# jipolanco/PencilArrays.jl

Hardware: NVIDIA H100
Metric: transpose_GiB_per_s (higher is better)
Workload: dtype c128 (bytes; pure data movement)

## Files before the change

pencilarrays.jl_b200/csrc/fft.cu:

```cuda
#include <cuda_runtime.h>

#include <algorithm>
#include <cmath>
#include <map>
#include <mutex>
#include <tuple>
#include <type_traits>
#include <vector>

#ifndef PA_FFT_TWIDDLE_LOOKUPS
#define PA_FFT_TWIDDLE_LOOKUPS 1
#endif
#include "fft_core.hpp"
#include "flags.cuh"
#include "pa_internal.hpp"

namespace pa {

using pa_fft::cplx;
using pa_fft::cplx_t;

template <class T>
struct Vec2;
template <>
struct Vec2<double> {
  using type = double2;
};
template <>
struct Vec2<float> {
  using type = float2;
};
__device__ __forceinline__ double2 vec2(double x, double y) { return make_double2(x, y); }
__device__ __forceinline__ float2 vec2(float x, float y) { return make_float2(x, y); }

template <class T, int STRIDE = 1>
struct Twiddles {
  const typename Vec2<T>::type* tab;
  __device__ __forceinline__ cplx_t<T> operator()(int k) const {
    const typename Vec2<T>::type w = __ldg(tab + STRIDE * k);
    return cplx_t<T>{w.x, w.y};
  }
};

constexpr int FFT_MAXB = 8;
constexpr int FFT_MAXO = PA_MAX_DIMS - 2;
constexpr int FFT_THREADS = 256;
constexpr int fft_lines(int logL) { return logL >= 10 ? 4 : 8; }
constexpr int fft_lines_f32(int logL) { return logL >= 10 ? 8 : 16; }

struct FftBlock {
  const char* src;
  int y0, ey;
  long long ssy;
  long long ssx;
  long long so[FFT_MAXO];
};
struct FftParams {
  int nb;
  FftBlock blk[FFT_MAXB];
  char* dst;
  long long ex;
  long long dsx;
  int no;
  long long oe[FFT_MAXO], dso[FFT_MAXO];
  int L, logL, sign, pitch;
  int linear;
  const void* tw;
  unsigned tiles_x;
  const void* tw4;
  int sine;
};

template <class T>
struct SmLine {
  cplx_t<T>* p;
  __device__ __forceinline__ cplx_t<T> get(int i) const { return p[pa_fft::pad_index(i)]; }
  __device__ __forceinline__ void put(int i, cplx_t<T> v) { p[pa_fft::pad_index(i)] = v; }
};

template <int LOGM>
struct PassRadix {
  static constexpr int LOGR = (LOGM % 3 == 0) ? 3 : (LOGM % 3);
};

template <int LOGL, int LOGM, int C, class T, class Tw>
__device__ __forceinline__ void fft_passes(cplx_t<T>* sm, int pitch, int ncol, int sign, const Tw& tw) {
  if constexpr (LOGM > 0) {
    constexpr int LOGR = PassRadix<LOGM>::LOGR;
    constexpr int R = 1 << LOGR, L = 1 << LOGL, M = 1 << LOGM;
    constexpr int PER_LINE = L / R;
    constexpr int TOTAL = C * PER_LINE;
#pragma unroll
    for (int w0 = 0; w0 < TOTAL; w0 += FFT_THREADS) {
      const int w = w0 + (int)threadIdx.x;
      const int c = w / PER_LINE, u = w % PER_LINE;
      if (w < TOTAL && c < ncol) {
        SmLine<T> x{sm + c * pitch};
        pa_fft::butterfly<R>(x, u, L, M, sign, tw);
      }
    }
    __syncthreads();
    fft_passes<LOGL, LOGM - LOGR, C>(sm, pitch, ncol, sign, tw);
  }
}

template <int LOGL, int LOGM>
__device__ __forceinline__ int fft_pos(int k) {
  if constexpr (LOGM == 0) {
    return 0;
  } else {
    constexpr int LOGR = PassRadix<LOGM>::LOGR;
    return ((k & ((1 << LOGR) - 1)) << (LOGM - LOGR)) + fft_pos<LOGL, LOGM - LOGR>(k >> LOGR);
  }
}

template <int LOGL, class T>
__device__ __forceinline__ T out_real(const T* line, int i) {
  return line[2 * pa_fft::pad_index(fft_pos<LOGL, LOGL>(i >> 1)) + (i & 1)];
}

template <int C, class T>
__device__ __forceinline__ void gather_rows(const FftParams& p, const long long* so_off, long long x0,
                                            int c, int r, int ncol, cplx_t<T>* line) {
  using V = typename Vec2<T>::type;
  constexpr int RS = FFT_THREADS / C;
  constexpr int U = 8;
#pragma unroll
  for (int b = 0; b < FFT_MAXB; ++b) {
    if (b < p.nb) {
      const FftBlock& B = p.blk[b];
      const char* s = B.src + so_off[b] + (x0 + c) * B.ssx;
      const int ey = B.ey, y0 = B.y0;
      const long long ssy = B.ssy;
      for (int y = r; y < ey; y += U * RS) {
        V v[U];
#pragma unroll
        for (int k = 0; k < U; ++k) {
          const int yy = y + k * RS;
          if (c < ncol && yy < ey) v[k] = __ldcs(reinterpret_cast<const V*>(s + (long long)yy * ssy));
        }
#pragma unroll
        for (int k = 0; k < U; ++k) {
          const int yy = y + k * RS;
          if (c < ncol && yy < ey) line[pa_fft::pad_index(y0 + yy)] = cplx_t<T>{v[k].x, v[k].y};
        }
      }
    }
  }
}

enum class RealMap {
  rfft,
  dct2,
  dct3,
};

template <RealMap MAP, int LOGL, class T>
__device__ __forceinline__ void put_real(T* line, int n, T x, bool sine) {
  constexpr int L = 1 << LOGL, N = 2 * L;
  if constexpr (MAP == RealMap::rfft) {
    line[2 * pa_fft::pad_index(n >> 1) + (n & 1)] = x;
  } else if constexpr (MAP == RealMap::dct2) {
    const int i = (n & 1) ? N - 1 - (n >> 1) : (n >> 1);
    line[2 * pa_fft::pad_index(i >> 1) + (i & 1)] = ((n & 1) && sine) ? -x : x;
  } else {
    const int j = sine ? N - 1 - n : n;
    if (j <= L) line[2 * pa_fft::pad_index(j)] = x;
    if (j >= L) line[2 * pa_fft::pad_index(N - j) + 1] = x;
  }
}

template <int C, class T, class Put>
__device__ __forceinline__ void gather_real_rows(const FftParams& p, const long long* so_off, long long x0,
                                                 int c, int r, int ncol, const Put& put) {
  constexpr int RS = FFT_THREADS / C;
  constexpr int U = 8;
#pragma unroll
  for (int b = 0; b < FFT_MAXB; ++b) {
    if (b < p.nb) {
      const FftBlock& B = p.blk[b];
      const char* s = B.src + so_off[b] + (x0 + c) * B.ssx;
      const int ey = B.ey, y0 = B.y0;
      const long long ssy = B.ssy;
      for (int y = r; y < ey; y += U * RS) {
        T v[U];
#pragma unroll
        for (int k = 0; k < U; ++k) {
          const int yy = y + k * RS;
          if (c < ncol && yy < ey) v[k] = __ldcs(reinterpret_cast<const T*>(s + (long long)yy * ssy));
        }
#pragma unroll
        for (int k = 0; k < U; ++k) {
          const int yy = y + k * RS;
          if (c < ncol && yy < ey) put(y0 + yy, v[k]);
        }
      }
    }
  }
}

__device__ __forceinline__ long long cta_offsets(const FftParams& p, int C, long long* so_off,
                                                 long long* d_off) {
  unsigned long long bid = blockIdx.x;
  const long long x0 = (long long)(bid % p.tiles_x) * C;
  bid /= p.tiles_x;
#pragma unroll
  for (int b = 0; b < FFT_MAXB; ++b) so_off[b] = 0;
  *d_off = 0;
#pragma unroll 1
  for (int i = 0; i < p.no; ++i) {
    const long long k = (long long)(bid % (unsigned long long)p.oe[i]);
    bid /= (unsigned long long)p.oe[i];
    *d_off += k * p.dso[i];
#pragma unroll
    for (int b = 0; b < FFT_MAXB; ++b)
      if (b < p.nb) so_off[b] += k * p.blk[b].so[i];
  }
  return x0;
}

template <int LOGL, int C, class T>
struct FftCtaShape {
  static constexpr int RS = FFT_THREADS / C;
  static constexpr int LOGRS = (C == 16) ? 4 : (C == 8) ? 5 : 6;
  static_assert((1 << LOGRS) == RS, "rows per sweep");
  static constexpr int LOGR1 = (sizeof(T) == 8 && C == 4 && LOGL > LOGRS) ? (LOGL - LOGRS) : 0;
  static_assert(LOGR1 == 0 || LOGL - LOGR1 == LOGRS, "first-pass stride must equal the sweep");
  static_assert(LOGR1 <= 4, "the register first pass is at most radix 16");
};

template <int LOGL, int C, class T>
__device__ __forceinline__ void fft_cta_lines(const FftParams& p, const long long* so_off, long long x0,
                                              int ncol, cplx_t<T>* sm) {
  using cx = cplx_t<T>;
  using V = typename Vec2<T>::type;
  constexpr int L = 1 << LOGL;
  const int t = threadIdx.x;
  const int pitch = p.pitch;

  constexpr int RS = FftCtaShape<LOGL, C, T>::RS;
  constexpr int LOGR1 = FftCtaShape<LOGL, C, T>::LOGR1;
  const V* twp = reinterpret_cast<const V*>(p.tw);
  const Twiddles<T> tw{twp};
  {
    const int c = p.linear ? t / RS : t % C, r = p.linear ? t % RS : t / C;
    cx* line = sm + c * pitch;
    if constexpr (LOGR1 > 0) {
      constexpr int R1 = 1 << LOGR1;
      if (c < ncol) {
        V v[R1];
#pragma unroll
        for (int q = 0; q < R1; ++q) {
          const int y = r + q * RS;
          const char* s = nullptr;
#pragma unroll
          for (int b = 0; b < FFT_MAXB; ++b)
            if (b < p.nb && y >= p.blk[b].y0 && y < p.blk[b].y0 + p.blk[b].ey)
              s = p.blk[b].src + so_off[b] + (long long)(y - p.blk[b].y0) * p.blk[b].ssy +
                  (x0 + c) * p.blk[b].ssx;
          v[q] = __ldcs(reinterpret_cast<const V*>(s));
        }
        cx a[R1];
#pragma unroll
        for (int q = 0; q < R1; ++q) a[q] = cx{v[q].x, v[q].y};
        pa_fft::butterfly_regs<R1>(a, r, L, L, p.sign, tw);
#pragma unroll
        for (int q = 0; q < R1; ++q) line[pa_fft::pad_index(r + q * RS)] = a[q];
      }
    } else {
      gather_rows<C, T>(p, so_off, x0, c, r, ncol, line);
    }
  }
  __syncthreads();

  fft_passes<LOGL, LOGL - LOGR1, C>(sm, pitch, ncol, p.sign, tw);
}

template <int LOGL, int LOGR1>
__device__ __forceinline__ int fft_out_pos(int k) {
  return ((k & ((1 << LOGR1) - 1)) << (LOGL - LOGR1)) + fft_pos<LOGL, LOGL - LOGR1>(k >> LOGR1);
}

template <int LOGL, int C, class T>
__device__ __forceinline__ void unpack_fft_cta(const FftParams& p) {
  using cx = cplx_t<T>;
  using V = typename Vec2<T>::type;
  constexpr int L = 1 << LOGL;
  extern __shared__ __align__(16) unsigned char fft_smem[];
  cx* sm = reinterpret_cast<cx*>(fft_smem);
  const int t = threadIdx.x;
  long long so_off[FFT_MAXB], d_off;
  const long long x0 = cta_offsets(p, C, so_off, &d_off);
  const int ncol = (int)((p.ex - x0) < C ? (p.ex - x0) : C);
  const int pitch = p.pitch;
  constexpr int LOGR1 = FftCtaShape<LOGL, C, T>::LOGR1;

  fft_cta_lines<LOGL, C, T>(p, so_off, x0, ncol, sm);

  char* d = p.dst + x0 * p.dsx + d_off;
  for (int c = 0; c < ncol; ++c) {
    const cx* line = sm + c * pitch;
    V* out = reinterpret_cast<V*>(d + c * p.dsx);
#pragma unroll
    for (int k0 = 0; k0 < L; k0 += FFT_THREADS) {
      const int k = k0 + t;
      if (k < L) {
        const int pos = ((k & ((1 << LOGR1) - 1)) << (LOGL - LOGR1)) +
                        fft_pos<LOGL, LOGL - LOGR1>(k >> LOGR1);
        const cx v = line[pa_fft::pad_index(pos)];
        __stcs(out + k, vec2(v.x, v.y));
      }
    }
  }
}

template <int LOGL, int C, class T>
__global__ void __launch_bounds__(FFT_THREADS) k_unpack_fft(const __grid_constant__ FftParams p) {
  unpack_fft_cta<LOGL, C, T>(p);
}

struct FftGetParams {
  FftParams p;
  MultiFlags mf;
};
static_assert(sizeof(FftGetParams) <= 4096, "FftParams + MultiFlags must fit the kernel parameters");

template <int LOGL, int C, class T>
__global__ void __maxnreg__(128) k_get_fft(const __grid_constant__ FftGetParams gp) {
  const MultiFlags& mf = gp.mf;
  if (mf.ready.n > 0) {
    if ((int)threadIdx.x < mf.ready.n) {
      if (blockIdx.x < 8) flag_signal(mf.ready.remote[threadIdx.x], mf.ready.seq[threadIdx.x]);
      flag_wait(mf.ready.local[threadIdx.x], mf.ready.seq[threadIdx.x], mf.timeout_ns, mf.err);
    }
    __syncthreads();
  }
  unpack_fft_cta<LOGL, C, T>(gp.p);
  if (mf.done.n > 0) {
    __syncthreads();
    int last = 0;
    if (threadIdx.x == 0) {
      __threadfence_system();
      last = atomicAdd(mf.counter, 1u) == gridDim.x - 1;
      if (last) {
        *mf.counter = 0;
        __threadfence_system();
      }
    }
    if (__syncthreads_or(last) && (int)threadIdx.x < mf.done.n)
      flag_signal(mf.done.remote[threadIdx.x], mf.done.seq[threadIdx.x]);
  }
}

struct RfftParams {
  const char* src;
  char* dst;
  long long nlines;
  long long src_line, dst_line;
  int pitch;
  const void* tw;
};

template <int LOGL, int C, class T, class Out>
__device__ __forceinline__ void rfft_forward_tail(cplx_t<T>* sm, int pitch, int ncol, int t,
                                                  const typename Vec2<T>::type* twp, const Out& out) {
  using cx = cplx_t<T>;
  using V = typename Vec2<T>::type;
  constexpr int L = 1 << LOGL;
  constexpr int P = L / 2 + 1;
  const Twiddles<T> twN{twp};
  const Twiddles<T, 2> twL{twp};
  fft_passes<LOGL, LOGL, C>(sm, pitch, ncol, -1, twL);

#pragma unroll
  for (int w0 = 0; w0 < C * P; w0 += FFT_THREADS) {
    const int w = w0 + t, c = w / P, k = w % P;
    if (w < C * P && c < ncol) {
      const cx* line = sm + c * pitch;
      cx xk, xl;
      pa_fft::rfft_post_pair(line[pa_fft::pad_index(fft_pos<LOGL, LOGL>(k & (L - 1)))],
                             line[pa_fft::pad_index(fft_pos<LOGL, LOGL>((L - k) & (L - 1)))], twN(k),
                             &xk, &xl);
      V* o = reinterpret_cast<V*>(out(c));
      __stcs(o + k, vec2(xk.x, xk.y));
      if (k != L - k) __stcs(o + (L - k), vec2(xl.x, xl.y));
    }
  }
}

template <int LOGL, int C, bool UNROLL, class T>
__device__ __forceinline__ void brfft_pre(cplx_t<T>* sm, int pitch, int ncol, int t, const Twiddles<T>& twN) {
  using cx = cplx_t<T>;
  constexpr int L = 1 << LOGL;
  constexpr int P = L / 2 + 1;
  constexpr int TRIPS = (C * P + FFT_THREADS - 1) / FFT_THREADS;
#pragma unroll(UNROLL ? TRIPS : 1)
  for (int w0 = 0; w0 < C * P; w0 += FFT_THREADS) {
    const int w = w0 + t, c = w / P, k = w % P;
    if (w < C * P && c < ncol) {
      cx* line = sm + c * pitch;
      cx zk, zl;
      pa_fft::brfft_pre_pair(k, line[pa_fft::pad_index(k)], line[pa_fft::pad_index(L - k)], twN(k),
                             &zk, &zl);
      line[pa_fft::pad_index(k)] = zk;
      if (k > 0) line[pa_fft::pad_index(L - k)] = zl;
    }
  }
  __syncthreads();
}

template <int LOGL, int C, bool FWD, class T, class Src>
__device__ __forceinline__ void rfft_load(cplx_t<T>* sm, int pitch, int ncol, int t, const Src& src) {
  using cx = cplx_t<T>;
  using V = typename Vec2<T>::type;
  constexpr int L = 1 << LOGL;
  constexpr int RS = FFT_THREADS / C;
  constexpr int NIN = FWD ? L : L + 1;
  constexpr int U = (NIN + RS - 1) / RS;
  const int c = t / RS, r = t % RS;
  if (c < ncol) {
    const V* s = src(c);
    cx* line = sm + c * pitch;
    V v[U];
#pragma unroll
    for (int q = 0; q < U; ++q)
      if (r + q * RS < NIN) v[q] = __ldcs(s + r + q * RS);
#pragma unroll
    for (int q = 0; q < U; ++q)
      if (r + q * RS < NIN) line[pa_fft::pad_index(r + q * RS)] = cx{v[q].x, v[q].y};
  }
}

template <int LOGL, int C, bool FWD, class T>
__global__ void __launch_bounds__(FFT_THREADS) k_rfft(const __grid_constant__ RfftParams p) {
  using cx = cplx_t<T>;
  using V = typename Vec2<T>::type;
  constexpr int L = 1 << LOGL;
  extern __shared__ __align__(16) unsigned char fft_smem[];
  cx* sm = reinterpret_cast<cx*>(fft_smem);
  const int t = threadIdx.x;
  const long long l0 = (long long)blockIdx.x * C;
  const int ncol = (int)((p.nlines - l0) < C ? (p.nlines - l0) : C);
  const int pitch = p.pitch;
  const V* twp = reinterpret_cast<const V*>(p.tw);

  rfft_load<LOGL, C, FWD, T>(sm, pitch, ncol, t, [&p, l0](int c) {
    return reinterpret_cast<const V*>(p.src + (l0 + c) * p.src_line);
  });
  __syncthreads();

  if constexpr (FWD) {
    rfft_forward_tail<LOGL, C, T>(sm, pitch, ncol, t, twp,
                                  [&p, l0](int c) { return p.dst + (l0 + c) * p.dst_line; });
  } else {
    brfft_pre<LOGL, C, true, T>(sm, pitch, ncol, t, Twiddles<T>{twp});
    fft_passes<LOGL, LOGL, C>(sm, pitch, ncol, 1, Twiddles<T, 2>{twp});

#pragma unroll
    for (int w0 = 0; w0 < C * L; w0 += FFT_THREADS) {
      const int w = w0 + t, c = w >> LOGL, n = w & (L - 1);
      if (c < ncol) {
        const cx v = sm[c * pitch + pa_fft::pad_index(fft_pos<LOGL, LOGL>(n))];
        __stcs(reinterpret_cast<V*>(p.dst + (l0 + c) * p.dst_line) + n, vec2(v.x, v.y));
      }
    }
  }
}

template <int LOGL, int C, class T>
__global__ void __launch_bounds__(FFT_THREADS) k_unpack_brfft(const __grid_constant__ FftParams p) {
  using cx = cplx_t<T>;
  using V = typename Vec2<T>::type;
  constexpr int L = 1 << LOGL;
  constexpr int RS = FFT_THREADS / C;
  extern __shared__ __align__(16) unsigned char fft_smem[];
  cx* sm = reinterpret_cast<cx*>(fft_smem);
  const int t = threadIdx.x;
  long long so_off[FFT_MAXB], d_off;
  const long long x0 = cta_offsets(p, C, so_off, &d_off);
  const int ncol = (int)((p.ex - x0) < C ? (p.ex - x0) : C);
  const int pitch = p.pitch;
// ... 147 lines not shown
  cx* sm = reinterpret_cast<cx*>(fft_smem);
  const int t = threadIdx.x;
  const long long l0 = (long long)blockIdx.x * C;
  const int ncol = (int)((p.nlines - l0) < C ? (p.nlines - l0) : C);
  const int pitch = p.pitch;
  const bool sine = p.sine != 0;
  const V* twp = reinterpret_cast<const V*>(p.tw);
  const V* tw4p = reinterpret_cast<const V*>(p.tw4);

  r2r_load<LOGL, C, FWD, T>(sm, pitch, ncol, t, sine, [&p, l0](int c) {
    return reinterpret_cast<const V*>(p.src + (l0 + c) * p.line);
  });
  __syncthreads();

  r2r_tail<LOGL, C, FWD, T>(sm, pitch, ncol, t, sine, twp, tw4p,
                            [&p, l0](int c) { return p.dst + (l0 + c) * p.line; });
}

template <int LOGL, int C, bool FWD, class T>
__global__ void __launch_bounds__(FFT_THREADS) k_unpack_r2r(const __grid_constant__ FftParams p) {
  using cx = cplx_t<T>;
  using V = typename Vec2<T>::type;
  constexpr int RS = FFT_THREADS / C;
  extern __shared__ __align__(16) unsigned char fft_smem[];
  cx* sm = reinterpret_cast<cx*>(fft_smem);
  const int t = threadIdx.x;
  long long so_off[FFT_MAXB], d_off;
  const long long x0 = cta_offsets(p, C, so_off, &d_off);
  const int ncol = (int)((p.ex - x0) < C ? (p.ex - x0) : C);
  const int pitch = p.pitch;
  const bool sine = p.sine != 0;

  {
    const int c = p.linear ? t / RS : t % C, r = p.linear ? t % RS : t / C;
    T* line = reinterpret_cast<T*>(sm + c * pitch);
    gather_real_rows<C, T>(p, so_off, x0, c, r, ncol, [line, sine](int n, T x) {
      put_real<FWD ? RealMap::dct2 : RealMap::dct3, LOGL>(line, n, x, sine);
    });
    if (!FWD && r == 0 && c < ncol) line[1] = T(0);
  }
  __syncthreads();

  char* d = p.dst + x0 * p.dsx + d_off;
  r2r_tail<LOGL, C, FWD, T>(sm, pitch, ncol, t, sine, reinterpret_cast<const V*>(p.tw),
                            reinterpret_cast<const V*>(p.tw4),
                            [&p, d](int c) { return d + c * p.dsx; });
}

template <int LOGL, int C, class T>
__global__ void __launch_bounds__(FFT_THREADS) k_unpack_rfft(const __grid_constant__ FftParams p) {
  using cx = cplx_t<T>;
  using V = typename Vec2<T>::type;
  constexpr int RS = FFT_THREADS / C;
  extern __shared__ __align__(16) unsigned char fft_smem[];
  cx* sm = reinterpret_cast<cx*>(fft_smem);
  const int t = threadIdx.x;
  long long so_off[FFT_MAXB], d_off;
  const long long x0 = cta_offsets(p, C, so_off, &d_off);
  const int ncol = (int)((p.ex - x0) < C ? (p.ex - x0) : C);
  const int pitch = p.pitch;

  {
    const int c = p.linear ? t / RS : t % C, r = p.linear ? t % RS : t / C;
    T* line = reinterpret_cast<T*>(sm + c * pitch);
    gather_real_rows<C, T>(p, so_off, x0, c, r, ncol,
                           [line](int n, T x) { put_real<RealMap::rfft, LOGL>(line, n, x, false); });
  }
  __syncthreads();

  char* d = p.dst + x0 * p.dsx + d_off;
  rfft_forward_tail<LOGL, C, T>(sm, pitch, ncol, t, reinterpret_cast<const V*>(p.tw),
                                [&p, d](int c) { return d + c * p.dsx; });
}

struct FftPutBlock {
  char* dst;
  int y0, ey;
  long long dsy;
  long long dsx;
  long long dso[FFT_MAXO];
};
struct FftPutParams {
  FftParams p;
  int nb;
  int across;
  FftPutBlock blk[FFT_MAXB];
  MultiFlags mf;
};
static_assert(sizeof(FftPutParams) <= 4096, "FftPutParams must fit the kernel parameters");

__device__ __forceinline__ void put_ready_signal(const MultiFlags& mf) {
  if (mf.ready.n > 0 && blockIdx.x < 8 && (int)threadIdx.x < mf.ready.n)
    flag_signal(mf.ready.remote[threadIdx.x], mf.ready.seq[threadIdx.x]);
}
__device__ __forceinline__ void put_ready_wait(const MultiFlags& mf) {
  if (mf.ready.n > 0) {
    if ((int)threadIdx.x < mf.ready.n)
      flag_wait(mf.ready.local[threadIdx.x], mf.ready.seq[threadIdx.x], mf.timeout_ns, mf.err);
    __syncthreads();
  }
}
__device__ __forceinline__ void put_done(const MultiFlags& mf) {
  if (mf.done.n > 0) {
    __syncthreads();
    int last = 0;
    if (threadIdx.x == 0) {
      __threadfence_system();
      last = atomicAdd(mf.counter, 1u) == gridDim.x - 1;
      if (last) {
        *mf.counter = 0;
        __threadfence_system();
      }
    }
    if (__syncthreads_or(last) && (int)threadIdx.x < mf.done.n) {
      flag_signal(mf.done.remote[threadIdx.x], mf.done.seq[threadIdx.x]);
      if (mf.wait_done) flag_wait(mf.done.local[threadIdx.x], mf.done.seq[threadIdx.x], mf.timeout_ns, mf.err);
    }
  }
}

template <class E>
__device__ __forceinline__ E* put_at(const FftPutParams& pp, char* const* base, int c, int k) {
  char* o = nullptr;
#pragma unroll
  for (int b = 0; b < FFT_MAXB; ++b)
    if (b < pp.nb && k >= pp.blk[b].y0 && k < pp.blk[b].y0 + pp.blk[b].ey)
      o = base[b] + (long long)(k - pp.blk[b].y0) * pp.blk[b].dsy + c * pp.blk[b].dsx;
  return reinterpret_cast<E*>(o);
}
template <class T>
__device__ __forceinline__ typename Vec2<T>::type* put_target(const FftPutParams& pp, char* const* base,
                                                              int c, int k) {
  return put_at<typename Vec2<T>::type>(pp, base, c, k);
}

__device__ __forceinline__ void put_bases(const FftPutParams& pp, long long x0, char** base) {
  long long off[FFT_MAXB];
#pragma unroll
  for (int b = 0; b < FFT_MAXB; ++b) off[b] = 0;
  unsigned long long bid = blockIdx.x / pp.p.tiles_x;
#pragma unroll 1
  for (int i = 0; i < pp.p.no; ++i) {
    const long long k = (long long)(bid % (unsigned long long)pp.p.oe[i]);
    bid /= (unsigned long long)pp.p.oe[i];
#pragma unroll
    for (int b = 0; b < FFT_MAXB; ++b)
      if (b < pp.nb) off[b] += k * pp.blk[b].dso[i];
  }
#pragma unroll
  for (int b = 0; b < FFT_MAXB; ++b) base[b] = pp.blk[b].dst + off[b] + x0 * pp.blk[b].dsx;
}

template <int LOGL, int C, class T>
__global__ void __maxnreg__(128) k_fft_put(const __grid_constant__ FftPutParams pp) {
  using cx = cplx_t<T>;
  constexpr int L = 1 << LOGL;
  constexpr int LOGR1 = FftCtaShape<LOGL, C, T>::LOGR1;
  extern __shared__ __align__(16) unsigned char fft_smem[];
  cx* sm = reinterpret_cast<cx*>(fft_smem);
  const FftParams& p = pp.p;
  const int t = threadIdx.x;
  put_ready_signal(pp.mf);
  long long so_off[FFT_MAXB], d_off;
  const long long x0 = cta_offsets(p, C, so_off, &d_off);
  const int ncol = (int)((p.ex - x0) < C ? (p.ex - x0) : C);
  fft_cta_lines<LOGL, C, T>(p, so_off, x0, ncol, sm);
  put_ready_wait(pp.mf);

  char* base[FFT_MAXB];
  put_bases(pp, x0, base);
  const bool across = pp.across != 0;
  for (int w0 = 0; w0 < C * L; w0 += FFT_THREADS) {
    const int w = w0 + t;
    const int c = across ? (w & (C - 1)) : (w >> LOGL), k = across ? (w / C) : (w & (L - 1));
    if (w < C * L && c < ncol) {
      const cx v = sm[c * p.pitch + pa_fft::pad_index(fft_out_pos<LOGL, LOGR1>(k))];
      __stcs(put_target<T>(pp, base, c, k), vec2(v.x, v.y));
    }
  }
  put_done(pp.mf);
}

template <int LOGL, int C, class T>
__global__ void __maxnreg__(128) k_rfft_put(const __grid_constant__ FftPutParams pp) {
  using cx = cplx_t<T>;
  using V = typename Vec2<T>::type;
  constexpr int L = 1 << LOGL;
  constexpr int P = L / 2 + 1;
  extern __shared__ __align__(16) unsigned char fft_smem[];
  cx* sm = reinterpret_cast<cx*>(fft_smem);
  const FftParams& p = pp.p;
  const int t = threadIdx.x;
  put_ready_signal(pp.mf);
  long long so_off[FFT_MAXB], d_off;
  const long long x0 = cta_offsets(p, C, so_off, &d_off);
  const int ncol = (int)((p.ex - x0) < C ? (p.ex - x0) : C);
  const int pitch = p.pitch;
  rfft_load<LOGL, C, true, T>(sm, pitch, ncol, t, [&p, &so_off, x0](int c) {
    return reinterpret_cast<const V*>(p.blk[0].src + so_off[0] + (x0 + c) * p.blk[0].ssx);
  });
  __syncthreads();
  const V* twp = reinterpret_cast<const V*>(p.tw);
  const Twiddles<T> twN{twp};
  const Twiddles<T, 2> twL{twp};
  fft_passes<LOGL, LOGL, C>(sm, pitch, ncol, -1, twL);
  put_ready_wait(pp.mf);

  char* base[FFT_MAXB];
  put_bases(pp, x0, base);
  const bool across = pp.across != 0;
  for (int w0 = 0; w0 < C * P; w0 += FFT_THREADS) {
    const int w = w0 + t;
    const int c = across ? (w & (C - 1)) : (w / P), k = across ? (w / C) : (w % P);
    if (w < C * P && c < ncol) {
      const cx* line = sm + c * pitch;
      cx xk, xl;
      pa_fft::rfft_post_pair(line[pa_fft::pad_index(fft_pos<LOGL, LOGL>(k & (L - 1)))],
                             line[pa_fft::pad_index(fft_pos<LOGL, LOGL>((L - k) & (L - 1)))], twN(k),
                             &xk, &xl);
      __stcs(put_target<T>(pp, base, c, k), vec2(xk.x, xk.y));
      if (k != L - k) __stcs(put_target<T>(pp, base, c, L - k), vec2(xl.x, xl.y));
    }
  }
  put_done(pp.mf);
}


template <int LOGL, int C, bool FWD, class T>
__global__ void __maxnreg__(128) k_r2r_put(const __grid_constant__ FftPutParams pp) {
  using cx = cplx_t<T>;
  using V = typename Vec2<T>::type;
  constexpr int L = 1 << LOGL, N = 2 * L;
  constexpr int P = L / 2 + 1;
  extern __shared__ __align__(16) unsigned char fft_smem[];
  cx* sm = reinterpret_cast<cx*>(fft_smem);
  const FftParams& p = pp.p;
  const int t = threadIdx.x;
  put_ready_signal(pp.mf);
  long long so_off[FFT_MAXB], d_off;
  const long long x0 = cta_offsets(p, C, so_off, &d_off);
  const int ncol = (int)((p.ex - x0) < C ? (p.ex - x0) : C);
  const int pitch = p.pitch;
  const bool sine = p.sine != 0;
  const V* twp = reinterpret_cast<const V*>(p.tw);
  const V* tw4p = reinterpret_cast<const V*>(p.tw4);
  r2r_load<LOGL, C, FWD, T>(sm, pitch, ncol, t, sine, [&p, &so_off, x0](int c) {
    return reinterpret_cast<const V*>(p.blk[0].src + so_off[0] + (x0 + c) * p.blk[0].ssx);
  });
  __syncthreads();
  const Twiddles<T, 2> twL{twp};
  if constexpr (!FWD) r2r_pre<LOGL, C, T>(sm, pitch, ncol, t, Twiddles<T>{twp}, Twiddles<T>{tw4p});
  fft_passes<LOGL, LOGL, C>(sm, pitch, ncol, FWD ? -1 : 1, twL);
  put_ready_wait(pp.mf);

  char* base[FFT_MAXB];
  put_bases(pp, x0, base);
  const bool across = pp.across != 0;
  if constexpr (FWD) {
    const Twiddles<T> twN{twp};
    const Twiddles<T> w4{tw4p};
    for (int w0 = 0; w0 < C * P; w0 += FFT_THREADS) {
      const int w = w0 + t;
      const int c = across ? (w & (C - 1)) : (w / P), k = across ? (w / C) : (w % P);
      if (w < C * P && c < ncol) {
        const cx* line = sm + c * pitch;
        cx vk, vl;
        pa_fft::rfft_post_pair(line[pa_fft::pad_index(fft_pos<LOGL, LOGL>(k & (L - 1)))],
                               line[pa_fft::pad_index(fft_pos<LOGL, LOGL>((L - k) & (L - 1)))], twN(k),
                               &vk, &vl);
        T yk, ynk, yl, ynl;
        pa_fft::dct2_post_pair(vk, w4(k), &yk, &ynk);
        pa_fft::dct2_post_pair(vl, w4(L - k), &yl, &ynl);
        auto put = [&](int j, T y) { __stcs(put_at<T>(pp, base, c, sine ? N - 1 - j : j), y); };
        put(k, yk);
        if (k > 0 && k < L / 2) put(N - k, ynk);
        if (k < L / 2) put(L - k, yl);
        if (k > 0) put(L + k, ynl);
      }
    }
  } else {
    for (int w0 = 0; w0 < C * N; w0 += FFT_THREADS) {
      const int w = w0 + t;
      const int c = across ? (w & (C - 1)) : (w >> (LOGL + 1)), n = across ? (w / C) : (w & (N - 1));
      if (w < C * N && c < ncol) {
        const T* line = reinterpret_cast<const T*>(sm + c * pitch);
        const int i = (n & 1) ? N - 1 - (n >> 1) : (n >> 1);
        const T v = out_real<LOGL>(line, i);
        __stcs(put_at<T>(pp, base, c, n), (sine && (n & 1)) ? -v : v);
      }
    }
  }
  put_done(pp.mf);
}

template <int LOGL, int C, class T>
__global__ void __maxnreg__(128) k_brfft_put(const __grid_constant__ FftPutParams pp) {
  using cx = cplx_t<T>;
  using V = typename Vec2<T>::type;
  constexpr int L = 1 << LOGL, N = 2 * L;
  extern __shared__ __align__(16) unsigned char fft_smem[];
  cx* sm = reinterpret_cast<cx*>(fft_smem);
  const FftParams& p = pp.p;
  const int t = threadIdx.x;
  put_ready_signal(pp.mf);
  long long so_off[FFT_MAXB], d_off;
  const long long x0 = cta_offsets(p, C, so_off, &d_off);
  const int ncol = (int)((p.ex - x0) < C ? (p.ex - x0) : C);
  const int pitch = p.pitch;
  rfft_load<LOGL, C, false, T>(sm, pitch, ncol, t, [&p, &so_off, x0](int c) {
    return reinterpret_cast<const V*>(p.blk[0].src + so_off[0] + (x0 + c) * p.blk[0].ssx);
  });
  __syncthreads();
  const V* twp = reinterpret_cast<const V*>(p.tw);
  const Twiddles<T> twN{twp};
  const Twiddles<T, 2> twL{twp};
  brfft_pre<LOGL, C, true, T>(sm, pitch, ncol, t, twN);
  fft_passes<LOGL, LOGL, C>(sm, pitch, ncol, 1, twL);
  put_ready_wait(pp.mf);

  char* base[FFT_MAXB];
  put_bases(pp, x0, base);
  const bool across = pp.across != 0;
  for (int w0 = 0; w0 < C * N; w0 += FFT_THREADS) {
    const int w = w0 + t;
    const int c = across ? (w & (C - 1)) : (w >> (LOGL + 1)), n = across ? (w / C) : (w & (N - 1));
    if (w < C * N && c < ncol) {
      const T* line = reinterpret_cast<const T*>(sm + c * pitch);
      __stcs(put_at<T>(pp, base, c, n), out_real<LOGL>(line, n));
    }
  }
  put_done(pp.mf);
}
// ... 763 lines not shown
```

Before: 1377.

## Fold first and last FFT radix passes into register gather and store

For double precision, the FFT line kernel now runs a register-resident first radix pass for more CTA shapes, not only C==4, and batches several butterflies per thread. The final radix-8 pass is fused into the output store, so each thread reads 8 elements from shared memory, applies the butterfly in registers and writes straight to global memory. This removes one shared-memory pass and one barrier at each end of the FFT. In exchange it adds register pressure and a strided store pattern, which is partly offset by a lane swizzle meant to keep writes coalesced. A profiling script comparing two builds is also added.

```diff
diff --git a/pencilarrays.jl_b200/csrc/fft.cu b/pencilarrays.jl_b200/csrc/fft.cu
--- a/pencilarrays.jl_b200/csrc/fft.cu
+++ b/pencilarrays.jl_b200/csrc/fft.cu
@@ -83,9 +83,9 @@
   static constexpr int LOGR = (LOGM % 3 == 0) ? 3 : (LOGM % 3);
 };
 
-template <int LOGL, int LOGM, int C, class T, class Tw>
+template <int LOGL, int LOGM, int C, int LOGEND = 0, class T, class Tw>
 __device__ __forceinline__ void fft_passes(cplx_t<T>* sm, int pitch, int ncol, int sign, const Tw& tw) {
-  if constexpr (LOGM > 0) {
+  if constexpr (LOGM > LOGEND) {
     constexpr int LOGR = PassRadix<LOGM>::LOGR;
     constexpr int R = 1 << LOGR, L = 1 << LOGL, M = 1 << LOGM;
     constexpr int PER_LINE = L / R;
@@ -100,7 +100,7 @@
       }
     }
     __syncthreads();
-    fft_passes<LOGL, LOGM - LOGR, C>(sm, pitch, ncol, sign, tw);
+    fft_passes<LOGL, LOGM - LOGR, C, LOGEND>(sm, pitch, ncol, sign, tw);
   }
 }
 
@@ -224,12 +224,16 @@
   static constexpr int RS = FFT_THREADS / C;
   static constexpr int LOGRS = (C == 16) ? 4 : (C == 8) ? 5 : 6;
   static_assert((1 << LOGRS) == RS, "rows per sweep");
-  static constexpr int LOGR1 = (sizeof(T) == 8 && C == 4 && LOGL > LOGRS) ? (LOGL - LOGRS) : 0;
-  static_assert(LOGR1 == 0 || LOGL - LOGR1 == LOGRS, "first-pass stride must equal the sweep");
+  static constexpr int LOGR1N = PassRadix<LOGL>::LOGR;
+  static constexpr int LOGR1 = sizeof(T) != 8             ? 0
+                               : (C == 4 && LOGL > LOGRS) ? (LOGL - LOGRS)
+                               : (LOGL - LOGR1N >= LOGRS) ? LOGR1N
+                                                          : 0;
+  static_assert(LOGR1 == 0 || LOGL - LOGR1 >= LOGRS, "first-pass stride must be whole sweeps");
   static_assert(LOGR1 <= 4, "the register first pass is at most radix 16");
 };
 
-template <int LOGL, int C, class T>
+template <int LOGL, int C, class T, int LOGEND = 0>
 __device__ __forceinline__ void fft_cta_lines(const FftParams& p, const long long* so_off, long long x0,
                                               int ncol, cplx_t<T>* sm) {
   using cx = cplx_t<T>;
@@ -246,26 +250,37 @@
     const int c = p.linear ? t / RS : t % C, r = p.linear ? t % RS : t / C;
     cx* line = sm + c * pitch;
     if constexpr (LOGR1 > 0) {
-      constexpr int R1 = 1 << LOGR1;
+      constexpr int R1 = 1 << LOGR1, S = L >> LOGR1;
+      constexpr int NBF = S / RS;
+      constexpr int G = (R1 >= 8) ? 1 : (NBF < 8 / R1 ? NBF : 8 / R1);
       if (c < ncol) {
-        V v[R1];
-#pragma unroll
-        for (int q = 0; q < R1; ++q) {
-          const int y = r + q * RS;
-          const char* s = nullptr;
-#pragma unroll
-          for (int b = 0; b < FFT_MAXB; ++b)
-            if (b < p.nb && y >= p.blk[b].y0 && y < p.blk[b].y0 + p.blk[b].ey)
-              s = p.blk[b].src + so_off[b] + (long long)(y - p.blk[b].y0) * p.blk[b].ssy +
-                  (x0 + c) * p.blk[b].ssx;
-          v[q] = __ldcs(reinterpret_cast<const V*>(s));
+#pragma unroll 1
+        for (int m0 = 0; m0 < NBF; m0 += G) {
+          V v[G][R1];
+#pragma unroll
+          for (int g = 0; g < G; ++g)
+#pragma unroll
+            for (int q = 0; q < R1; ++q) {
+              const int y = r + (m0 + g) * RS + q * S;
+              const char* s = nullptr;
+#pragma unroll
+              for (int b = 0; b < FFT_MAXB; ++b)
+                if (b < p.nb && y >= p.blk[b].y0 && y < p.blk[b].y0 + p.blk[b].ey)
+                  s = p.blk[b].src + so_off[b] + (long long)(y - p.blk[b].y0) * p.blk[b].ssy +
+                      (x0 + c) * p.blk[b].ssx;
+              v[g][q] = __ldcs(reinterpret_cast<const V*>(s));
+            }
+#pragma unroll
+          for (int g = 0; g < G; ++g) {
+            const int j = r + (m0 + g) * RS;
+            cx a[R1];
+#pragma unroll
+            for (int q = 0; q < R1; ++q) a[q] = cx{v[g][q].x, v[g][q].y};
+            pa_fft::butterfly_regs<R1>(a, j, L, L, p.sign, tw);
+#pragma unroll
+            for (int q = 0; q < R1; ++q) line[pa_fft::pad_index(j + q * S)] = a[q];
+          }
         }
-        cx a[R1];
-#pragma unroll
-        for (int q = 0; q < R1; ++q) a[q] = cx{v[q].x, v[q].y};
-        pa_fft::butterfly_regs<R1>(a, r, L, L, p.sign, tw);
-#pragma unroll
-        for (int q = 0; q < R1; ++q) line[pa_fft::pad_index(r + q * RS)] = a[q];
       }
     } else {
       gather_rows<C, T>(p, so_off, x0, c, r, ncol, line);
@@ -273,7 +288,7 @@
   }
   __syncthreads();
 
-  fft_passes<LOGL, LOGL - LOGR1, C>(sm, pitch, ncol, p.sign, tw);
+  fft_passes<LOGL, LOGL - LOGR1, C, LOGEND>(sm, pitch, ncol, p.sign, tw);
 }
 
 template <int LOGL, int LOGR1>
@@ -295,20 +310,44 @@
   const int pitch = p.pitch;
   constexpr int LOGR1 = FftCtaShape<LOGL, C, T>::LOGR1;
 
-  fft_cta_lines<LOGL, C, T>(p, so_off, x0, ncol, sm);
-
-  char* d = p.dst + x0 * p.dsx + d_off;
-  for (int c = 0; c < ncol; ++c) {
-    const cx* line = sm + c * pitch;
-    V* out = reinterpret_cast<V*>(d + c * p.dsx);
-#pragma unroll
-    for (int k0 = 0; k0 < L; k0 += FFT_THREADS) {
-      const int k = k0 + t;
-      if (k < L) {
-        const int pos = ((k & ((1 << LOGR1) - 1)) << (LOGL - LOGR1)) +
-                        fft_pos<LOGL, LOGL - LOGR1>(k >> LOGR1);
-        const cx v = line[pa_fft::pad_index(pos)];
-        __stcs(out + k, vec2(v.x, v.y));
+  if constexpr (sizeof(T) == 8) {
+    const Twiddles<T> tw{reinterpret_cast<const V*>(p.tw)};
+    fft_cta_lines<LOGL, C, T, 3>(p, so_off, x0, ncol, sm);
+    char* d = p.dst + x0 * p.dsx + d_off;
+    constexpr int NG = L / 8, TOTAL = C * NG;
+    const int lane = t & 31;
+    const int wt = (t & ~31) | (LOGR1 == 4 ? lane : ((lane & 7) << 2) | (lane >> 3));
+#pragma unroll 1
+    for (int w0 = 0; w0 < TOTAL; w0 += FFT_THREADS) {
+      const int w = w0 + wt;
+      const int c = w / NG, i = w % NG;
+      if (w < TOTAL && c < ncol) {
+        const cx* x = sm + c * pitch + pa_fft::pad_index(fft_out_pos<LOGL, LOGR1>(i));
+        cx a[8];
+#pragma unroll
+        for (int q = 0; q < 8; ++q) a[q] = x[q];
+        pa_fft::butterfly_regs<8>(a, 0, L, 8, p.sign, tw);
+        V* out = reinterpret_cast<V*>(d + c * p.dsx) + i;
+#pragma unroll
+        for (int s = 0; s < 8; ++s) __stcs(out + s * NG, vec2(a[s].x, a[s].y));
+      }
+    }
+  } else {
+    fft_cta_lines<LOGL, C, T>(p, so_off, x0, ncol, sm);
+
+    char* d = p.dst + x0 * p.dsx + d_off;
+    for (int c = 0; c < ncol; ++c) {
+      const cx* line = sm + c * pitch;
+      V* out = reinterpret_cast<V*>(d + c * p.dsx);
+#pragma unroll
+      for (int k0 = 0; k0 < L; k0 += FFT_THREADS) {
+        const int k = k0 + t;
+        if (k < L) {
+          const int pos = ((k & ((1 << LOGR1) - 1)) << (LOGL - LOGR1)) +
+                          fft_pos<LOGL, LOGL - LOGR1>(k >> LOGR1);
+          const cx v = line[pa_fft::pad_index(pos)];
+          __stcs(out + k, vec2(v.x, v.y));
+        }
       }
     }
   }
diff --git a/profiles/prof_fft_regpass.py b/profiles/prof_fft_regpass.py
--- /dev/null
+++ b/profiles/prof_fft_regpass.py
@@ -0,0 +1,190 @@
+#!/usr/bin/env python
+import argparse
+import ctypes as C
+import hashlib
+import json
+import os
+import statistics
+import subprocess
+import sys
+import tempfile
+
+HERE = os.path.dirname(os.path.abspath(__file__))
+REPS = 20
+
+
+def child(root, out):
+    sys.path.insert(0, os.path.abspath(root))
+    import torch
+    import pencilarrays_b200 as pa
+    from pencilarrays_b200 import _lib
+    from pencilarrays_b200._lib import lib, check
+    from pencilarrays_b200.transpositions import _Plan
+
+    assert pa.__file__.startswith(os.path.abspath(root)), pa.__file__
+    torch.cuda.set_device(0)
+    real = {torch.complex128: torch.float64, torch.complex64: torch.float32}
+
+    def seeded(u):
+        v = u.data.view(real[u.data.dtype])
+        g = torch.Generator(device="cuda").manual_seed(1234)
+        v.copy_(torch.randn(v.shape, generator=g, device="cuda", dtype=v.dtype))
+
+    def digest(ts):
+        acc = []
+        for t in ts:
+            v = t.contiguous().view(torch.int64).reshape(-1)
+            w = torch.arange(v.numel(), device=v.device, dtype=torch.int64) * -7046029254386353131 + 1
+            acc += [int((v * w).sum()), int(((v ^ (v >> 17)) * w).sum())]
+            del w
+        return hashlib.sha256(repr(acc).encode()).hexdigest()[:16]
+
+    def timed(fn):
+        for _ in range(3):
+            fn()
+        a, b = torch.cuda.Event(enable_timing=True), torch.cuda.Event(enable_timing=True)
+        a.record()
+        for _ in range(REPS):
+            fn()
+        b.record()
+        torch.cuda.synchronize()
+        return a.elapsed_time(b) / REPS
+
+    topo = pa.MPITopology(pa.COMM_SELF, (1, 1))
+    res = {}
+
+    def transposing(name, dims, dtype, leg):
+        px = pa.Pencil(topo, dims, (2, 3))
+        py = pa.Pencil(px, decomp_dims=(1, 3), permute=pa.Permutation(2, 1, 3))
+        pz = pa.Pencil(py, decomp_dims=(1, 2), permute=pa.Permutation(3, 2, 1))
+        pi, po = (px, py) if leg == "xy" else (py, pz)
+        ui, uo = pa.PencilArray.undef(dtype, pi), pa.PencilArray.undef(dtype, po)
+        t = pa.Transposition(uo, ui)
+        sha = {}
+        for d in ("forward", "backward"):
+            seeded(ui)
+            pa.transpose_(t, fft=d)
+            torch.cuda.synchronize()
+            sha[d] = digest([uo.data])
+        seeded(ui)
+        res[name] = dict(ms=timed(lambda: pa.transpose_(t, fft="forward")), sha=sha)
+
+    def inplace(name, dims, dtype):
+        u = pa.PencilArray.undef(dtype, pa.Pencil(topo, dims, (2, 3)))
+        sha = {}
+        for d in ("forward", "backward"):
+            seeded(u)
+            pa.fft_(u, d)
+            torch.cuda.synchronize()
+            sha[d] = digest([u.data])
+        res[name] = dict(ms=timed(lambda: pa.fft_(u, "forward")), sha=sha)
+
+    def emulated(name, dims, dtype, R=2):
+        es = 16 if dtype == torch.complex128 else 8
+        f32 = 0 if dtype == torch.complex128 else _lib.PA_FFT_F32
+        put, get, src, dst = [], [], [], []
+        for r in range(R):
+            tp = pa.MPITopology(pa.Comm(r, R), (R,))
+            px = pa.Pencil(tp, dims, (2,))
+            py = pa.Pencil(px, decomp_dims=(1,), permute=pa.Permutation(2, 1, 3))
+            put.append(_Plan(px, py, (), es, pa.PeerPut()))
+            get.append(_Plan(px, py, (), es, pa.PeerGet()))
+            src.append(pa.PencilArray.undef(dtype, px))
+            dst.append(pa.PencilArray.undef(dtype, py))
+        ptrs = lambda ts: (C.c_void_p * len(ts))(*[t.data_ptr() for t in ts])
+        dst_all = [ptrs([dst[pl.peer(k).world_rank] for k in range(1, R + 1)]) for pl in put]
+        src_all = [ptrs([src[pl.peer(k).world_rank] for k in range(1, R + 1)]) for pl in get]
+
+        def run_put(flag):
+            st = C.c_void_p(torch.cuda.current_stream().cuda_stream)
+            for r, pl in enumerate(put):
+                check(lib.pa_put_all_fft(pl.h, C.c_void_p(src[r].data_ptr()), dst_all[r],
+                                         C.c_void_p(dst[r].data_ptr()), flag | f32, st))
+
+        def run_get(flag):
+            st = C.c_void_p(torch.cuda.current_stream().cuda_stream)
+            for r, pl in enumerate(get):
+                check(lib.pa_get_all_fft(pl.h, C.c_void_p(src[r].data_ptr()), src_all[r],
+                                         C.c_void_p(dst[r].data_ptr()), flag | f32, st))
+
+        check(lib.pa_set_device(torch.cuda.current_device()))
+        for kind, run in (("put", run_put), ("get", run_get)):
+            sha = {}
+            for d, flag in (("forward", _lib.PA_FFT_FORWARD), ("backward", _lib.PA_FFT_BACKWARD)):
+                for u in src:
+                    seeded(u)
+                run(flag)
+                torch.cuda.synchronize()
+                sha[d] = digest([u.data for u in dst])
+            res[f"{name} {kind}"] = dict(ms=timed(lambda: run(_lib.PA_FFT_FORWARD)), sha=sha)
+
+    n512 = (512, 512, 512)
+    for dtype, tag in ((torch.complex128, "c128"), (torch.complex64, "c64")):
+        transposing(f"x->y 512^3 {tag} (bench fused_fft shape)" if tag == "c128" else f"x->y 512^3 {tag}",
+                    n512, dtype, "xy")
+        transposing(f"y->z 512^3 {tag}", n512, dtype, "yz")
+        transposing(f"x->y 512x1024x256 {tag} (1024-point lines)", (512, 1024, 256), dtype, "xy")
+        for L in (256, 512):
+            inplace(f"fft_ L={L} {tag} ({L}x512x512)", (L, 512, 512), dtype)
+        emulated(f"2-rank emulated 512^3 {tag}", n512, dtype)
+        torch.cuda.empty_cache()
+    json.dump(res, open(out, "w"))
+
+
+def card():
+    import torch
+    name = torch.cuda.get_device_name(0)
+    try:
+        q = subprocess.run(["nvidia-smi", "--query-gpu=power.limit,clocks.max.sm", "--format=csv,noheader",
+                            "-i", "0"], capture_output=True, text=True, timeout=30)
+        return name, q.stdout.strip()
+    except Exception as e:
+        return name, f"unknown ({e})"
+
+
+def main():
+    ap = argparse.ArgumentParser()
+    ap.add_argument("--a", default=os.path.join(os.path.dirname(HERE), "build", "ab_parent"),
+                    help="tree of build A (default: build/ab_parent)")
+    ap.add_argument("--b", default=os.path.dirname(HERE), help="tree of build B (default: this tree)")
+    ap.add_argument("--alts", type=int, default=5, help="turns of each build (>= 5 for a spread)")
+    ap.add_argument("--json", default=None)
+    ap.add_argument("--child", default=None, help=argparse.SUPPRESS)
+    ap.add_argument("--out", default=None, help=argparse.SUPPRESS)
+    args = ap.parse_args()
+    if args.child:
+        return child(args.child, args.out)
+    name, power = card()
+    print(f"card: {name}; power.limit, clocks.max.sm: {power}", flush=True)
+    runs = {"A": [], "B": []}
+    with tempfile.TemporaryDirectory() as tmp:
+        for i in range(args.alts):
+            for lab, root in (("A", args.a), ("B", args.b)):
+                out = os.path.join(tmp, f"{lab}{i}.json")
+                subprocess.run([sys.executable, os.path.abspath(__file__), "--child", root, "--out", out],
+                               check=True)
+                runs[lab].append(json.load(open(out)))
+                print(f"turn {i} {lab} done", flush=True)
+    rows = [dict(card=name, power_limit_and_max_sm_clock=power, a=args.a, b=args.b, alts=args.alts, reps=REPS)]
+    all_equal = True
+    for case in runs["A"][0]:
+        row = dict(case=case)
+        for lab in ("A", "B"):
+            ms = [r[case]["ms"] for r in runs[lab]]
+            row[lab] = dict(median_ms=round(statistics.median(ms), 4), min_ms=round(min(ms), 4),
+                            max_ms=round(max(ms), 4))
+        shas = {(lab, d): r[case]["sha"][d] for lab in ("A", "B") for r in runs[lab] for d in ("forward", "backward")}
+        row["bytes_equal"] = all(runs["A"][0][case]["sha"][d] == s for (lab, d), s in shas.items())
+        all_equal &= row["bytes_equal"]
+        row["speedup"] = round(row["A"]["median_ms"] / row["B"]["median_ms"], 3)
+        row["spreads_overlap"] = not (row["B"]["max_ms"] < row["A"]["min_ms"] or row["A"]["max_ms"] < row["B"]["min_ms"])
+        rows.append(row)
+        print(json.dumps(row), flush=True)
+    print("outputs byte-identical between the builds:", all_equal, flush=True)
+    if args.json:
+        json.dump(rows, open(args.json, "w"), indent=1)
+    return 0 if all_equal else 1
+
+
+if __name__ == "__main__":
+    sys.exit(main())
```

Result: no change. 1376, median of 6 (-0.0%).

## Fuse final radix-8 FFT pass into store and widen register first pass

Applied to the files above, without the earlier changes.

For double-precision complex data, the last radix-8 butterfly pass is now done in registers while values are written to global memory. This removes one shared-memory pass and one barrier. The register first pass is extended to more lengths and cta shapes, with grouped batched loads to give more memory parallelism. Launch bounds now set a minimum CTA count per SM instead of a fixed 128-register cap, which may cause spills or change occupancy.

```diff
diff --git a/pencilarrays.jl_b200/csrc/fft.cu b/pencilarrays.jl_b200/csrc/fft.cu
--- a/pencilarrays.jl_b200/csrc/fft.cu
+++ b/pencilarrays.jl_b200/csrc/fft.cu
@@ -83,9 +83,9 @@
   static constexpr int LOGR = (LOGM % 3 == 0) ? 3 : (LOGM % 3);
 };
 
-template <int LOGL, int LOGM, int C, class T, class Tw>
+template <int LOGL, int LOGM, int C, class T, class Tw, int LOGEND = 0>
 __device__ __forceinline__ void fft_passes(cplx_t<T>* sm, int pitch, int ncol, int sign, const Tw& tw) {
-  if constexpr (LOGM > 0) {
+  if constexpr (LOGM > LOGEND) {
     constexpr int LOGR = PassRadix<LOGM>::LOGR;
     constexpr int R = 1 << LOGR, L = 1 << LOGL, M = 1 << LOGM;
     constexpr int PER_LINE = L / R;
@@ -100,7 +100,7 @@
       }
     }
     __syncthreads();
-    fft_passes<LOGL, LOGM - LOGR, C>(sm, pitch, ncol, sign, tw);
+    fft_passes<LOGL, LOGM - LOGR, C, T, Tw, LOGEND>(sm, pitch, ncol, sign, tw);
   }
 }
 
@@ -224,9 +224,16 @@
   static constexpr int RS = FFT_THREADS / C;
   static constexpr int LOGRS = (C == 16) ? 4 : (C == 8) ? 5 : 6;
   static_assert((1 << LOGRS) == RS, "rows per sweep");
-  static constexpr int LOGR1 = (sizeof(T) == 8 && C == 4 && LOGL > LOGRS) ? (LOGL - LOGRS) : 0;
-  static_assert(LOGR1 == 0 || LOGL - LOGR1 == LOGRS, "first-pass stride must equal the sweep");
+  static constexpr int LOGRN = PassRadix<LOGL>::LOGR;
+  static constexpr bool REGS = sizeof(T) == 8;
+  static constexpr int LOGR1 = !REGS                                                  ? 0
+                               : (C == 4 && LOGL == 10)                               ? 4
+                               : (LOGL - LOGRN >= LOGRS && LOGL - LOGRN <= LOGRS + 2) ? LOGRN
+                                                                                      : 0;
+  static_assert(LOGR1 == 0 || LOGL - LOGR1 >= LOGRS, "first-pass stride must be a multiple of the sweep");
   static_assert(LOGR1 <= 4, "the register first pass is at most radix 16");
+  static constexpr int NB1 = LOGR1 > 0 ? 1 << (LOGL - LOGR1 - LOGRS) : 0;
+  static constexpr int MIN_CTAS = LOGL < 8 ? (sizeof(T) == 8 ? 4 : 3) : (sizeof(T) == 4 || C == 8) ? 3 : 2;
 };
 
 template <int LOGL, int C, class T>
@@ -246,26 +253,37 @@
     const int c = p.linear ? t / RS : t % C, r = p.linear ? t % RS : t / C;
     cx* line = sm + c * pitch;
     if constexpr (LOGR1 > 0) {
-      constexpr int R1 = 1 << LOGR1;
+      constexpr int R1 = 1 << LOGR1, Q1 = L >> LOGR1;
+      constexpr int NB1 = FftCtaShape<LOGL, C, T>::NB1;
+      constexpr int G = R1 >= 8 ? 1 : (NB1 < 8 / R1 ? NB1 : 8 / R1);
       if (c < ncol) {
-        V v[R1];
-#pragma unroll
-        for (int q = 0; q < R1; ++q) {
-          const int y = r + q * RS;
-          const char* s = nullptr;
-#pragma unroll
-          for (int b = 0; b < FFT_MAXB; ++b)
-            if (b < p.nb && y >= p.blk[b].y0 && y < p.blk[b].y0 + p.blk[b].ey)
-              s = p.blk[b].src + so_off[b] + (long long)(y - p.blk[b].y0) * p.blk[b].ssy +
-                  (x0 + c) * p.blk[b].ssx;
-          v[q] = __ldcs(reinterpret_cast<const V*>(s));
+#pragma unroll
+        for (int m0 = 0; m0 < NB1; m0 += G) {
+          V v[G][R1];
+#pragma unroll
+          for (int g = 0; g < G; ++g)
+#pragma unroll
+            for (int q = 0; q < R1; ++q) {
+              const int y = r + (m0 + g) * RS + q * Q1;
+              const char* s = nullptr;
+#pragma unroll
+              for (int b = 0; b < FFT_MAXB; ++b)
+                if (b < p.nb && y >= p.blk[b].y0 && y < p.blk[b].y0 + p.blk[b].ey)
+                  s = p.blk[b].src + so_off[b] + (long long)(y - p.blk[b].y0) * p.blk[b].ssy +
+                      (x0 + c) * p.blk[b].ssx;
+              v[g][q] = __ldcs(reinterpret_cast<const V*>(s));
+            }
+#pragma unroll
+          for (int g = 0; g < G; ++g) {
+            const int u = r + (m0 + g) * RS;
+            cx a[R1];
+#pragma unroll
+            for (int q = 0; q < R1; ++q) a[q] = cx{v[g][q].x, v[g][q].y};
+            pa_fft::butterfly_regs<R1>(a, u, L, L, p.sign, tw);
+#pragma unroll
+            for (int q = 0; q < R1; ++q) line[pa_fft::pad_index(u + q * Q1)] = a[q];
+          }
         }
-        cx a[R1];
-#pragma unroll
-        for (int q = 0; q < R1; ++q) a[q] = cx{v[q].x, v[q].y};
-        pa_fft::butterfly_regs<R1>(a, r, L, L, p.sign, tw);
-#pragma unroll
-        for (int q = 0; q < R1; ++q) line[pa_fft::pad_index(r + q * RS)] = a[q];
       }
     } else {
       gather_rows<C, T>(p, so_off, x0, c, r, ncol, line);
@@ -273,49 +291,70 @@
   }
   __syncthreads();
 
-  fft_passes<LOGL, LOGL - LOGR1, C>(sm, pitch, ncol, p.sign, tw);
+  fft_passes<LOGL, LOGL - LOGR1, C, T, Twiddles<T>, (FftCtaShape<LOGL, C, T>::REGS ? 3 : 0)>(sm, pitch, ncol,
+                                                                                          p.sign, tw);
 }
 
 template <int LOGL, int LOGR1>
 __device__ __forceinline__ int fft_out_pos(int k) {
   return ((k & ((1 << LOGR1) - 1)) << (LOGL - LOGR1)) + fft_pos<LOGL, LOGL - LOGR1>(k >> LOGR1);
+}
+
+template <int LOGL, int C, class T, class Out>
+__device__ __forceinline__ void fft_last_pass_store(const cplx_t<T>* sm, int pitch, int ncol, int sign,
+                                                    bool across, const Out& out) {
+  using cx = cplx_t<T>;
+  constexpr int LOGG = LOGL - 3, G = 1 << LOGG;
+  constexpr int LOGR1 = FftCtaShape<LOGL, C, T>::LOGR1;
+  const int t = threadIdx.x;
+  if constexpr (!FftCtaShape<LOGL, C, T>::REGS) {
+    constexpr int L = 1 << LOGL;
+    for (int w0 = 0; w0 < C * L; w0 += FFT_THREADS) {
+      const int w = w0 + t;
+      const int c = across ? (w & (C - 1)) : (w >> LOGL), k = across ? (w / C) : (w & (L - 1));
+      if (w < C * L && c < ncol) {
+        const cx v = sm[c * pitch + pa_fft::pad_index(fft_out_pos<LOGL, 0>(k))];
+        __stcs(out(c, k), vec2(v.x, v.y));
+      }
+    }
+    return;
+  }
+#pragma unroll
+  for (int w0 = 0; w0 < C * G; w0 += FFT_THREADS) {
+    const int w = w0 + t;
+    const int c = across ? (w & (C - 1)) : (w >> LOGG), kl = across ? (w / C) : (w & (G - 1));
+    if (w < C * G && c < ncol) {
+      const cx* line = sm + c * pitch;
+      const int base = fft_out_pos<LOGL, LOGR1>(kl);
+      cx a[8];
+#pragma unroll
+      for (int q = 0; q < 8; ++q) a[q] = line[pa_fft::pad_index(base + q)];
+      pa_fft::dft8(a, sign);
+#pragma unroll
+      for (int s = 0; s < 8; ++s) __stcs(out(c, kl + s * G), vec2(a[s].x, a[s].y));
+    }
+  }
 }
 
 template <int LOGL, int C, class T>
 __device__ __forceinline__ void unpack_fft_cta(const FftParams& p) {
   using cx = cplx_t<T>;
   using V = typename Vec2<T>::type;
-  constexpr int L = 1 << LOGL;
   extern __shared__ __align__(16) unsigned char fft_smem[];
   cx* sm = reinterpret_cast<cx*>(fft_smem);
-  const int t = threadIdx.x;
   long long so_off[FFT_MAXB], d_off;
   const long long x0 = cta_offsets(p, C, so_off, &d_off);
   const int ncol = (int)((p.ex - x0) < C ? (p.ex - x0) : C);
-  const int pitch = p.pitch;
-  constexpr int LOGR1 = FftCtaShape<LOGL, C, T>::LOGR1;
 
   fft_cta_lines<LOGL, C, T>(p, so_off, x0, ncol, sm);
 
   char* d = p.dst + x0 * p.dsx + d_off;
-  for (int c = 0; c < ncol; ++c) {
-    const cx* line = sm + c * pitch;
-    V* out = reinterpret_cast<V*>(d + c * p.dsx);
-#pragma unroll
-    for (int k0 = 0; k0 < L; k0 += FFT_THREADS) {
-      const int k = k0 + t;
-      if (k < L) {
-        const int pos = ((k & ((1 << LOGR1) - 1)) << (LOGL - LOGR1)) +
-                        fft_pos<LOGL, LOGL - LOGR1>(k >> LOGR1);
-        const cx v = line[pa_fft::pad_index(pos)];
-        __stcs(out + k, vec2(v.x, v.y));
-      }
-    }
-  }
+  fft_last_pass_store<LOGL, C, T>(sm, p.pitch, ncol, p.sign, false,
+                                  [&p, d](int c, int k) { return reinterpret_cast<V*>(d + c * p.dsx) + k; });
 }
 
 template <int LOGL, int C, class T>
-__global__ void __launch_bounds__(FFT_THREADS) k_unpack_fft(const __grid_constant__ FftParams p) {
+__global__ void __launch_bounds__(FFT_THREADS, (FftCtaShape<LOGL, C, T>::MIN_CTAS)) k_unpack_fft(const __grid_constant__ FftParams p) {
   unpack_fft_cta<LOGL, C, T>(p);
 }
 
@@ -326,7 +365,7 @@
 static_assert(sizeof(FftGetParams) <= 4096, "FftParams + MultiFlags must fit the kernel parameters");
 
 template <int LOGL, int C, class T>
-__global__ void __maxnreg__(128) k_get_fft(const __grid_constant__ FftGetParams gp) {
+__global__ void __launch_bounds__(FFT_THREADS, (FftCtaShape<LOGL, C, T>::MIN_CTAS)) k_get_fft(const __grid_constant__ FftGetParams gp) {
   const MultiFlags& mf = gp.mf;
   if (mf.ready.n > 0) {
     if ((int)threadIdx.x < mf.ready.n) {
@@ -780,14 +819,12 @@
 }
 
 template <int LOGL, int C, class T>
-__global__ void __maxnreg__(128) k_fft_put(const __grid_constant__ FftPutParams pp) {
+__global__ void __launch_bounds__(FFT_THREADS, (sizeof(T) == 8 ? 2 : FftCtaShape<LOGL, C, T>::MIN_CTAS))
+    k_fft_put(const __grid_constant__ FftPutParams pp) {
   using cx = cplx_t<T>;
-  constexpr int L = 1 << LOGL;
-  constexpr int LOGR1 = FftCtaShape<LOGL, C, T>::LOGR1;
   extern __shared__ __align__(16) unsigned char fft_smem[];
   cx* sm = reinterpret_cast<cx*>(fft_smem);
   const FftParams& p = pp.p;
-  const int t = threadIdx.x;
   put_ready_signal(pp.mf);
   long long so_off[FFT_MAXB], d_off;
   const long long x0 = cta_offsets(p, C, so_off, &d_off);
@@ -797,15 +834,8 @@
 
   char* base[FFT_MAXB];
   put_bases(pp, x0, base);
-  const bool across = pp.across != 0;
-  for (int w0 = 0; w0 < C * L; w0 += FFT_THREADS) {
-    const int w = w0 + t;
-    const int c = across ? (w & (C - 1)) : (w >> LOGL), k = across ? (w / C) : (w & (L - 1));
-    if (w < C * L && c < ncol) {
-      const cx v = sm[c * p.pitch + pa_fft::pad_index(fft_out_pos<LOGL, LOGR1>(k))];
-      __stcs(put_target<T>(pp, base, c, k), vec2(v.x, v.y));
-    }
-  }
+  fft_last_pass_store<LOGL, C, T>(sm, p.pitch, ncol, p.sign, pp.across != 0,
+                                  [&pp, &base](int c, int k) { return put_target<T>(pp, base, c, k); });
   put_done(pp.mf);
 }
 
```

Result: no change. 1376 before, 1377 after (median of 6 runs) (+0.0%).
